# Canleskis/ephemeris-explorer

Measured on AMD Instinct MI355X. Metric: body-steps/s, higher is better.
Workload: dtype f64

## Files before the change

ephemeris_explorer_amd/build.py:

```python
import os
import subprocess
import sys
from pathlib import Path

HERE = Path(__file__).resolve().parent
CSRC = HERE / "csrc"
LIB = HERE / "libephemeris_amd.so"
HOOKS_LIB = HERE / "libephemeris_amd_testhooks.so"
HOOKS_SOURCES = ["debug_api.cpp", "debug_kernels.hip"]
N_PAIR_VARIANTS = 7
PAIR_SOURCES = ["step_wg.hip", "step_wave.hip", "step_small.hip", "step_double_small.hip", "step_srkn_small.hip", "fast.hip", "craft_sweep.hip"]
SOURCES = ["solout.hip", "double_step.hip", "craft.hip", "craft_events.hip", "ephemeris_table.hip", "evaluators.hip", "craft_eval.hip", "craft_restart.hip", "craft_gather.hip", "craft_plot.hip", "craft_markers.hip", "craft_separation.hip", "peer.hip", "dispatch.cpp", "mem.cpp", "coeffs.cpp", "nbody.cpp", "propagator.cpp", "shard.cpp", "api.cpp"]
EXPORTS = CSRC / "exports.map"
HEADERS = sorted(p.name for pat in ("*.h", "*.inc", "exports.map") for p in CSRC.glob(pat)) + ["../../include/ephemeris_amd.h"]
FLAGS = ["--offload-arch=gfx950", "-O3", "-std=c++17", "-fPIC", "-ffp-contract=off", "-fno-fast-math", "-fvisibility=hidden",
         "-Wall", "-Wno-unused-function", "-Wno-unused-result"]
FLAGS += os.environ.get("EPH_EXTRA_FLAGS", "").split()


def hipcc():
    for c in (os.environ.get("HIPCC"), "/opt/rocm/bin/hipcc", "hipcc"):
        if c and (os.path.isabs(c) and os.path.exists(c) or not os.path.isabs(c)):
            return c
    return "hipcc"


def units():
    out = [(src, CSRC / (src.rsplit(".", 1)[0] + ".o"), []) for src in SOURCES + HOOKS_SOURCES]
    for k in range(N_PAIR_VARIANTS):
        out += [(src, CSRC / (src.rsplit(".", 1)[0] + f".pv{k}.o"), [f"-DEPH_PAIR_VARIANT={k}"]) for src in PAIR_SOURCES]
    return out


def needs_build(lib=LIB):
    if not lib.exists():
        return True
    t = lib.stat().st_mtime
    return any((CSRC / f).stat().st_mtime > t for f in SOURCES + HOOKS_SOURCES + PAIR_SOURCES + HEADERS) or Path(__file__).stat().st_mtime > t


def build(force=False, verbose=False, lib=LIB, extra_flags=(), obj_dir=None, jobs=None):
    hooks = lib.with_name(lib.name.replace("libephemeris_amd", "libephemeris_amd_testhooks")) if lib == LIB else None
    if not force and not extra_flags and not needs_build(lib) and (hooks is None or not needs_build(hooks)):
        return lib
    from concurrent.futures import ThreadPoolExecutor
    newest_header = max((CSRC / h).stat().st_mtime for h in HEADERS)
    newest_header = max(newest_header, Path(__file__).stat().st_mtime)
    todo, objs = [], []
    for src, obj, fl in units():
        if obj_dir is not None:
            obj = Path(obj_dir) / obj.name
        objs.append(str(obj))
        if force or extra_flags or not obj.exists() or obj.stat().st_mtime < max((CSRC / src).stat().st_mtime, newest_header):
            todo.append((src, obj, fl))

    def compile_one(job):
        src, obj, fl = job
        cmd = [hipcc(), *FLAGS, *fl, *extra_flags, "-x", "hip", "-c", str(CSRC / src), "-o", str(obj)]
        if verbose:
            print(" ".join(cmd), file=sys.stderr)
        p = subprocess.run(cmd, stdout=subprocess.PIPE, stderr=subprocess.STDOUT)
        if p.returncode:
            raise RuntimeError(f"hipcc failed on {src} {' '.join(fl)}:\n{p.stdout.decode()}")
        if verbose and p.stdout:
            print(p.stdout.decode(), file=sys.stderr)

    todo.sort(key=lambda j: -(CSRC / j[0]).stat().st_size)
    with ThreadPoolExecutor(jobs or max(2, (os.cpu_count() or 4))) as ex:
        list(ex.map(compile_one, todo))
    hook_objs = [o for o in objs if Path(o).name in {h.rsplit(".", 1)[0] + ".o" for h in HOOKS_SOURCES}]
    link = [hipcc(), "--offload-arch=gfx950", "-shared", "-fPIC", f"-Wl,--version-script={EXPORTS}"]
    if hooks is not None:
        subprocess.check_call([*link, "-o", str(lib), *[o for o in objs if o not in hook_objs]])
        subprocess.check_call([*link, "-o", str(hooks), *objs])
    else:
        subprocess.check_call([*link, "-o", str(lib), *objs])
    return lib


def build_all(force=False, verbose=False):
    return [build(force, verbose), HOOKS_LIB]


if __name__ == "__main__":
    if "--exp" in sys.argv:
        i = sys.argv.index("--exp")
        name, flags = sys.argv[i + 1], sys.argv[i + 2:]
        od = Path("/tmp") / f"eph_exp_{name}"
        od.mkdir(parents=True, exist_ok=True)
        print(build(force=True, verbose=False, lib=HERE / f"libephemeris_amd_exp_{name}.so", extra_flags=flags, obj_dir=od))
    else:
        print(build(force="--force" in sys.argv, verbose="--verbose" in sys.argv))
```

ephemeris_explorer_amd/csrc/step_wg.hip:

```cpp
#include <algorithm>
#include <type_traits>
#include <utility>

#include "pair_ns.h"

#ifndef EPH_EXPERIMENTS
#define EPH_EXPERIMENTS 0
#endif
#if !EPH_EXPERIMENTS || !defined(EPH_WG_SIDE)
#undef EPH_WG_SIDE
#define EPH_WG_SIDE 0
#endif
#if !EPH_EXPERIMENTS || !defined(EPH_WG_ABLATE)
#undef EPH_WG_ABLATE
#define EPH_WG_ABLATE 0
#endif
#define WG_LOOP_BARRIER() do { if constexpr (!(EPH_WG_ABLATE & 2)) __syncthreads(); } while (0)


namespace eph {
namespace EPH_PV_NS {

constexpr int kWgBodies = 16;
constexpr int kDuoThreads = 64 * 6;
constexpr int kDuoTailWave = 5;
constexpr int kWgChainWave = 4;
constexpr int kWgTailWave = 8;
constexpr int kWgThreads = 64 * 12;
constexpr int kWgTileBufs = 6;
constexpr int kWgSplitBufs = 3;

template <int NB, int BS = 1, typename PosPtr>
__device__ __forceinline__ void wg_load_own(PosPtr pos, int n, int first, double (&xi)[NB], double (&yi)[NB], double (&zi)[NB]) {
#pragma unroll
    for (int b = 0; b < NB; ++b) {
        const int ii = min(first + BS * b, n - 1);
        xi[b] = pos[ii].x;
        yi[b] = pos[ii].y;
        zi[b] = pos[ii].z;
    }
}
template <typename PosPtr>
__device__ __forceinline__ Body4 load_src(PosPtr pos, int n, int tiles, int lane, int t) {
    const int j = min(t, tiles - 1) * kTile + lane;
    return pos[j < n ? j : n - 1];
}

template <int NB>
__device__ __forceinline__ void wg_pair_tile(const double (&xi)[NB], const double (&yi)[NB], const double (&zi)[NB],
                                             const Body4 &pj, bool ieee, double *tile, int b0, int lane) {
    PairPre pre[NB];
    unsigned worst = ieee ? kRangeSpan : mu_key(pj.mu), low = ~0u;
#pragma unroll
    for (int b = 0; b < NB; ++b) {
        pre[b] = pair_pre(xi[b], yi[b], zi[b], pj);
        worst = max(worst, range_key(pre[b].n2));
        low = min(low, pre[b].lo);
    }
    worst = max(worst, low_key(low));
    double c[3 * NB];
    if (__builtin_amdgcn_ballot_w64(worst >= kRangeSpan) == 0) {
#pragma unroll
        for (int b = 0; b < NB; ++b) pair_finish<true>(pre[b], pj.mu, c[3 * b], c[3 * b + 1], c[3 * b + 2]);
    } else {
#pragma unroll
        for (int b = 0; b < NB; ++b) pair_finish<false>(pre[b], pj.mu, c[3 * b], c[3 * b + 1], c[3 * b + 2]);
    }
#pragma unroll
    for (int q = 0; q < 3 * NB; ++q) {
        if constexpr (EPH_WG_ABLATE & 1) asm volatile("" ::"v"(c[q]));
        else tile[(3 * b0 + q) * kRow + lane] = c[q];
    }
}

template <int NB, typename PosPtr>
__device__ __forceinline__ void wg_pair_wave(PosPtr pos, int n, int i0, int b0, double *C, int lane, int tiles, int tdiag, int wbuf) {
    double xi[NB], yi[NB], zi[NB];
    wg_load_own<NB>(pos, n, i0 + b0, xi, yi, zi);
    Body4 pj = load_src(pos, n, tiles, lane, 0);
    Body4 pjn = load_src(pos, n, tiles, lane, 1);
    wg_pair_tile<NB>(xi, yi, zi, pj, tdiag == 0, C, b0, lane);
    pj = pjn;
    pjn = load_src(pos, n, tiles, lane, 2);
    if (tiles > 1) wg_pair_tile<NB>(xi, yi, zi, pj, tdiag == 1, C + wbuf, b0, lane);
    __syncthreads();
    for (int t = 0; t < tiles; ++t) {
        if (t + 2 < tiles) {
            pj = pjn;
            pjn = load_src(pos, n, tiles, lane, t + 3);
            wg_pair_tile<NB>(xi, yi, zi, pj, tdiag == t + 2, C + ((t + 2) % kWgSplitBufs) * wbuf, b0, lane);
        }
        __syncthreads();
    }
}

template <int NB>
__device__ __forceinline__ void wg_pair_tile2(const double (&xi)[NB], const double (&yi)[NB], const double (&zi)[NB],
                                              const Body4 &pa, const Body4 &pb, bool ieee, double *tile_a, double *tile_b,
                                              int b0, int lane) {
    PairPre pre[2 * NB];
    unsigned worst = ieee ? kRangeSpan : max(mu_key(pa.mu), mu_key(pb.mu)), low = ~0u;
#pragma unroll
    for (int b = 0; b < NB; ++b) {
        pre[b] = pair_pre(xi[b], yi[b], zi[b], pa);
        pre[NB + b] = pair_pre(xi[b], yi[b], zi[b], pb);
        worst = max(worst, max(range_key(pre[b].n2), range_key(pre[NB + b].n2)));
        low = min(low, min(pre[b].lo, pre[NB + b].lo));
    }
    worst = max(worst, low_key(low));
    double c[6 * NB];
    if (__builtin_amdgcn_ballot_w64(worst >= kRangeSpan) == 0) {
        if constexpr (kPairStaged) {
            double mus[2 * NB];
#pragma unroll
            for (int b = 0; b < NB; ++b) { mus[b] = pa.mu; mus[NB + b] = pb.mu; }
            pair_finish_staged<2 * NB>(pre, mus, c);
        } else {
#pragma unroll
            for (int b = 0; b < NB; ++b) {
                pair_finish<true>(pre[b], pa.mu, c[3 * b], c[3 * b + 1], c[3 * b + 2]);
                pair_finish<true>(pre[NB + b], pb.mu, c[3 * (NB + b)], c[3 * (NB + b) + 1], c[3 * (NB + b) + 2]);
            }
        }
    } else {
#pragma unroll
        for (int b = 0; b < NB; ++b) {
            pair_finish<false>(pre[b], pa.mu, c[3 * b], c[3 * b + 1], c[3 * b + 2]);
            pair_finish<false>(pre[NB + b], pb.mu, c[3 * (NB + b)], c[3 * (NB + b) + 1], c[3 * (NB + b) + 2]);
        }
    }
#pragma unroll
    for (int q = 0; q < 3 * NB; ++q) {
        if constexpr (EPH_WG_ABLATE & 1) {
            asm volatile("" ::"v"(c[q]), "v"(c[3 * NB + q]));
        } else {
            tile_a[(3 * b0 + q) * kRow + lane] = c[q];
            tile_b[(3 * b0 + q) * kRow + lane] = c[3 * NB + q];
        }
    }
}

__device__ __forceinline__ int big_start(int K) { return K < 2 ? K : 2 * K - 2; }
__device__ __forceinline__ int big_count(int tiles) { return tiles <= 2 ? tiles : 2 + (tiles - 2 + 1) / 2; }
template <int NB, typename PosPtr>
__device__ __forceinline__ void wg_pair_wave_big(PosPtr pos, int n, int i0, int b0, double *C, int lane, int tiles, int tdiag, int wbuf) {
    double xi[NB], yi[NB], zi[NB];
#pragma unroll
    for (int b = 0; b < NB; ++b) {
        const int ii = min(i0 + b0 + b, n - 1);
        xi[b] = pos[ii].x;
        yi[b] = pos[ii].y;
        zi[b] = pos[ii].z;
    }
    auto produce = [&](int K, const Body4 &pa, const Body4 &pb) {
        const int t = big_start(K);
        if (t >= tiles || EPH_WG_SIDE == 2) return;
        double *ta = C + (t % kWgTileBufs) * wbuf, *tb = C + ((t + 1) % kWgTileBufs) * wbuf;
        if (K >= 2 && t + 1 < tiles) wg_pair_tile2<NB>(xi, yi, zi, pa, pb, tdiag == t || tdiag == t + 1, ta, tb, b0, lane);
        else wg_pair_tile<NB>(xi, yi, zi, pa, tdiag == t, ta, b0, lane);
    };
    const int TB = big_count(tiles);
    Body4 pa = load_src(pos, n, tiles, lane, 0), pb = load_src(pos, n, tiles, lane, 1);
    Body4 na = load_src(pos, n, tiles, lane, 2), nb = load_src(pos, n, tiles, lane, 3);
    produce(0, pa, pa);
    produce(1, pb, pb);
    __syncthreads();
    for (int K = 0; K < TB; ++K) {
        pa = na; pb = nb;
        na = load_src(pos, n, tiles, lane, big_start(K + 3));
        nb = load_src(pos, n, tiles, lane, big_start(K + 3) + 1);
        produce(K + 2, pa, pb);
        WG_LOOP_BARRIER();
    }
}
__device__ __forceinline__ void wg_idle_wave(int tiles) {
    __syncthreads();
    for (int T = 0; T < big_count(tiles); ++T) WG_LOOP_BARRIER();
}

constexpr bool kWgLateThird = kPairVariant == 0 || kPairVariant == 4 || kPairVariant == 5;
static_assert(kWgTileBufs == 6, "the late third tile needs tile t + 6 to be written two intervals after tile t was read");
__device__ __forceinline__ int phase_start(int P) { return P < 2 ? P : 3 * P - 4; }
__device__ __forceinline__ int phase_count(int tiles) { return tiles <= 2 ? tiles : 2 + (tiles - 2 + 2) / 3; }
__device__ __forceinline__ int phase_tiles(int P, int tiles) { return P < 2 ? 1 : min(3, tiles - phase_start(P)); }
__device__ __forceinline__ int interval_count(int tiles) { return phase_count(tiles) + (kWgLateThird && tiles >= 5 && (tiles - 2) % 3 == 0); }
__device__ __forceinline__ int chain_first(int I) { return kWgLateThird ? (I <= 2 ? I : 3 * I - 5) : phase_start(I); }

template <int MA, int MB>
__device__ __forceinline__ void pair_finish_staged_split(const PairPre (&pre)[MA + MB], const double (&mu)[MA + MB], double (&c)[3 * (MA + MB)]) {
    PairPre pa[MA], pb[MB];
    double ma[MA], mb[MB], ca[3 * MA], cb[3 * MB];
#pragma unroll
    for (int k = 0; k < MA; ++k) { pa[k] = pre[k]; ma[k] = mu[k]; }
#pragma unroll
    for (int k = 0; k < MB; ++k) { pb[k] = pre[MA + k]; mb[k] = mu[MA + k]; }
    pair_finish_staged<MA>(pa, ma, ca);
    pair_finish_staged<MB>(pb, mb, cb);
#pragma unroll
    for (int k = 0; k < 3 * MA; ++k) c[k] = ca[k];
#pragma unroll
    for (int k = 0; k < 3 * MB; ++k) c[3 * MA + k] = cb[k];
}

template <int NB, int BS>
__device__ __forceinline__ void wg_store_held(double *tile, int b0, int lane, const double (&held)[3 * NB]) {
#pragma unroll
    for (int q = 0; q < 3 * NB; ++q) {
        if constexpr (EPH_WG_ABLATE & 1) asm volatile("" ::"v"(held[q]));
        else tile[(3 * (b0 + BS * (q / 3)) + q % 3) * kRow + lane] = held[q];
    }
}

template <int NB, int NT, int BS = 1, bool LATE = false>
__device__ __forceinline__ void wg_pair_block(const double (&xi)[NB], const double (&yi)[NB], const double (&zi)[NB],
                                              const Body4 (&pj)[NT], bool ieee, double *const (&tile)[NT], int b0, int lane,
                                              double (&held)[3 * NB], double *held_tile) {
    constexpr int M = NB * NT;
    if constexpr (LATE) wg_store_held<NB, BS>(held_tile, b0, lane, held);
    PairPre pre[M];
    double mus[M];
    unsigned worst = ieee ? kRangeSpan : 0u, low = ~0u;
#pragma unroll
    for (int s = 0; s < NT; ++s) {
        worst = max(worst, mu_key(pj[s].mu));
#pragma unroll
        for (int b = 0; b < NB; ++b) {
            const int k = s * NB + b;
            pre[k] = pair_pre(xi[b], yi[b], zi[b], pj[s]);
            mus[k] = pj[s].mu;
            worst = max(worst, range_key(pre[k].n2));
            low = min(low, pre[k].lo);
        }
    }
    worst = max(worst, low_key(low));
    double c[3 * M];
    if (__builtin_amdgcn_ballot_w64(worst >= kRangeSpan) == 0) {
        if constexpr (kPairStaged && M == 5 && (kPairVariant == 4 || kPairVariant == 6)) {
            pair_finish_staged_split<3, 2>(pre, mus, c);
        } else if constexpr (kPairStaged) {
            pair_finish_staged<M>(pre, mus, c);
        } else {
#pragma unroll
            for (int k = 0; k < M; ++k) pair_finish<true>(pre[k], mus[k], c[3 * k], c[3 * k + 1], c[3 * k + 2]);
        }
    } else {
#pragma unroll
        for (int k = 0; k < M; ++k) pair_finish<false>(pre[k], mus[k], c[3 * k], c[3 * k + 1], c[3 * k + 2]);
    }
#pragma unroll
    for (int s = 0; s < NT - LATE; ++s) {
#pragma unroll
        for (int q = 0; q < 3 * NB; ++q) {
            if constexpr (EPH_WG_ABLATE & 1) asm volatile("" ::"v"(c[3 * NB * s + q]));
            else tile[s][(3 * (b0 + BS * (q / 3)) + q % 3) * kRow + lane] = c[3 * NB * s + q];
        }
    }
    if constexpr (LATE) {
#pragma unroll
        for (int q = 0; q < 3 * NB; ++q) held[q] = c[3 * NB * (NT - 1) + q];
    }
}
template <int NB, int NT, int BS = 1>
__device__ __forceinline__ void wg_pair_block(const double (&xi)[NB], const double (&yi)[NB], const double (&zi)[NB],
                                              const Body4 (&pj)[NT], bool ieee, double *const (&tile)[NT], int b0, int lane) {
    double none[3 * NB];
    wg_pair_block<NB, NT, BS, false>(xi, yi, zi, pj, ieee, tile, b0, lane, none, nullptr);
}

template <int NB, int BS = 1, typename PosPtr>
__device__ __forceinline__ void wg_pair_wave_deal(PosPtr pos, int n, int i0, int b0, int rank, double *C, int lane, int tiles, int tdiag, int wbuf) {
    double xi[NB], yi[NB], zi[NB];
    wg_load_own<NB, BS>(pos, n, i0 + b0, xi, yi, zi);
    auto tile_of = [&](int P) { return P < 2 ? (rank == 0 ? P : tiles) : phase_start(P) + rank; };
    constexpr bool kOff = EPH_WG_SIDE == 2 || (EPH_WG_SIDE == 3 && BS == 1);
    const int NI = interval_count(tiles);
    [[maybe_unused]] const int NP = kWgLateThird ? phase_count(tiles) : NI;
    if constexpr (NB == 5 || !kWgLateThird) {
        auto produce = [&](int t, const Body4 &pj) {
            if (t >= tiles || kOff) return;
            const Body4 src[1] = {pj};
            double *const dst[1] = {C + (t % kWgTileBufs) * wbuf};
            wg_pair_block<NB, 1, BS>(xi, yi, zi, src, t == tdiag, dst, b0, lane);
        };
        Body4 pj = load_src(pos, n, tiles, lane, tile_of(0)), pjn = load_src(pos, n, tiles, lane, tile_of(1));
        produce(tile_of(0), pj);
        __syncthreads();
        for (int P = 1; P < NP; ++P) {
            pj = pjn;
            pjn = load_src(pos, n, tiles, lane, tile_of(P + 1));
            produce(tile_of(P), pj);
            WG_LOOP_BARRIER();
        }
        if (NI > NP) WG_LOOP_BARRIER();
    } else {
        static_assert(NB < 5, "the late loop is the rank-2 waves' (four bodies) and wave 8's (three)");
        double held[3 * NB];
#pragma unroll
        for (int q = 0; q < 3 * NB; ++q) held[q] = 0.0;
        int tprev = tile_of(2);
        Body4 pj, pjn = load_src(pos, n, tiles, lane, tile_of(2));
        __syncthreads();
        for (int I = 1; I < NI; ++I) {
            const int t = I < 2 ? tiles : tile_of(I);
            if (I >= 2) {
                pj = pjn;
                pjn = load_src(pos, n, tiles, lane, tile_of(I + 1));
            }
            double *const late = C + (tprev % kWgTileBufs) * wbuf;
            if (kOff) {
            } else if (t < tiles) {
                const Body4 src[1] = {pj};
                double *const dst[1] = {nullptr};
                wg_pair_block<NB, 1, BS, true>(xi, yi, zi, src, t == tdiag, dst, b0, lane, held, late);
                tprev = t;
            } else if (tprev < tiles && I > 2) {
                wg_store_held<NB, BS>(late, b0, lane, held);
                tprev = tiles;
            }
            WG_LOOP_BARRIER();
        }
    }
}
template <typename PosPtr>
__device__ __forceinline__ void wg_pair_wave_solo(PosPtr pos, int n, int i0, double *C, int lane, int tiles, int tdiag, int wbuf) {
    double xi[1], yi[1], zi[1];
    wg_load_own<1>(pos, n, i0, xi, yi, zi);
    auto load_phase = [&](int P, Body4 (&s)[3]) {
        const int t = phase_start(P);
        s[0] = load_src(pos, n, tiles, lane, t);
        if (P >= 2) { s[1] = load_src(pos, n, tiles, lane, t + 1); s[2] = load_src(pos, n, tiles, lane, t + 2); }
    };
    const int NI = interval_count(tiles), NP = kWgLateThird ? phase_count(tiles) : NI;
    double held[3] = {0.0, 0.0, 0.0};
    int tprev = tiles;
    auto write_held = [&]() {
        if (tprev >= tiles) return;
        double *const late = C + (tprev % kWgTileBufs) * wbuf;
        wg_store_held<1, 1>(late, 0, lane, held);
        tprev = tiles;
    };
    auto produce = [&](int P, const Body4 (&s)[3]) {
        if (EPH_WG_SIDE == 2) return;
        if (P >= NP) { write_held(); return; }
        const int t = phase_start(P), cnt = phase_tiles(P, tiles);
        if (cnt == 3) {
            double *const dst[3] = {C + (t % kWgTileBufs) * wbuf, C + ((t + 1) % kWgTileBufs) * wbuf,
                                    kWgLateThird ? nullptr : C + ((t + 2) % kWgTileBufs) * wbuf};
            const bool below = tdiag < t + 3, own = tdiag >= t && below;
            double *const late = C + ((tprev < tiles ? tprev : t + 2) % kWgTileBufs) * wbuf;
            wg_pair_block<1, 3, 1, kWgLateThird>(xi, yi, zi, s, own, dst, 0, lane, held, late);
            if constexpr (kWgLateThird) tprev = t + 2;
        } else {
            write_held();
            auto one = [&](int k, const Body4 &pj) {
                const Body4 src[1] = {pj};
                double *const dst[1] = {C + ((t + k) % kWgTileBufs) * wbuf};
                wg_pair_block<1, 1>(xi, yi, zi, src, tdiag == t + k, dst, 0, lane);
            };
            one(0, s[0]);
            if (cnt > 1) one(1, s[1]);
        }
    };
    Body4 s[3], sn[3];
    load_phase(0, s);
    load_phase(1, sn);
    produce(0, s);
    __syncthreads();
    for (int P = 1; P < NI; ++P) {
#pragma unroll
        for (int k = 0; k < 3; ++k) s[k] = sn[k];
        load_phase(P + 1, sn);
        produce(P, s);
        WG_LOOP_BARRIER();
    }
}

__device__ __forceinline__ double chain_full_q(const double *row, double2 (&q)[4][8], double acc) {
    load_chunk(row, 2, q[2]);
    acc = add_chunk(q[0], acc);
    load_chunk(row, 3, q[3]);
    acc = add_chunk(q[1], acc);
    acc = add_chunk(q[2], acc);
    return add_chunk(q[3], acc);
}
__device__ __forceinline__ double chain_full_pf(const double *row, const double *row_next, double2 (&q)[4][8],
                                                double acc) {
    load_chunk(row, 2, q[2]);
    acc = add_chunk(q[0], acc);
    load_chunk(row, 3, q[3]);
    acc = add_chunk(q[1], acc);
    load_chunk(row_next, 0, q[0]);
    acc = add_chunk(q[2], acc);
    load_chunk(row_next, 1, q[1]);
    return add_chunk(q[3], acc);
}

constexpr bool wg_tile_split(int wb) { return wb == 4; }
constexpr int wg_split_wave_b(int wb) { return wb == 8 ? 11 : 6; }
template <int WB>
__device__ __forceinline__ int wg_small_body(int wave) {
    if constexpr (WB == 8) {
        switch (wave) { case 1: return 0; case 2: return 1; case 3: return 2; case 5: return 3; case 6: return 4; case 7: return 5;
                        case 9: return 6; case 10: return 7; default: return -1; }
    } else {
        switch (wave) { case 1: return 0; case 2: return 1; case 3: return 2; case 5: return 3; default: return -1; }
    }
}
template <int WB, typename PosPtr>
__device__ __forceinline__ double wg_force_split(PosPtr pos, int n, int i0, double init, double *C, int tid) {
    constexpr int kRows = 3 * WB, kBuf = kRows * kRow;
    const int lane = tid & 63, wave = tid >> 6;
    const int tiles = (n + kTile - 1) / kTile;
    const int tdiag = i0 / kTile;
    double *H = C + kWgSplitBufs * kBuf;
    const int body = wg_small_body<WB>(wave);
    if (body >= 0) { wg_pair_wave<1>(pos, n, i0, body, C, lane, tiles, tdiag, kBuf); return 0.0; }
    const bool isA = wave == kWgChainWave, isB = wave == wg_split_wave_b(WB);
    if (!isA && !isB) { for (int t = 0; t <= tiles; ++t) __syncthreads(); return 0.0; }
    const int ch = lane < kRows ? lane : kRows - 1;
    const double *row = C + ch * kRow;
    const int gself = (i0 % kTile) / WB;
    const int li = (i0 % kTile) + ch / 3;
    double acc = init, accL = 0.0;
    double2 q[4][8];
    auto plain = [&](int t) { return t < tiles && t != tdiag && min(kTile, n - t * kTile) == kTile; };
    auto preload = [&](int t) {
        const double *r = row + (t % kWgSplitBufs) * kBuf;
        load_chunk(r, 0, q[0]); load_chunk(r, 1, q[1]); load_chunk(r, 2, q[2]); load_chunk(r, 3, q[3]);
    };
    __syncthreads();
    if (isA && plain(0)) preload(0);
    for (int t = 0; t < tiles; ++t) {
        const bool mine = ((t & 1) != 0) == isB;
        if (mine) {
            if (t > 0) { acc = H[lane]; accL = H[64 + lane]; }
            if (plain(t)) {
                acc = add_chunk(q[0], acc); acc = add_chunk(q[1], acc); acc = add_chunk(q[2], acc); acc = add_chunk(q[3], acc);
            } else {
                chain_masked<WB>(row + (t % kWgSplitBufs) * kBuf, min(kTile, n - t * kTile), t == tdiag ? gself : -1, li, acc, accL);
            }
            H[lane] = acc;
            H[64 + lane] = accL;
        } else if (plain(t + 1)) {
            preload(t + 1);
        }
        __syncthreads();
    }
    return isA ? H[64 + lane] + H[lane] : 0.0;
}

constexpr int kWgShedFirst = 5, kWgShedStride = 5, kWgShedBodies = 3;
template <typename PosPtr>
__device__ __forceinline__ void wg_tail_wave_phases(PosPtr pos, int n, int i0, double *C, int lane, int tiles, int tdiag, int wbuf) {
    wg_pair_wave_deal<kWgShedBodies, kWgShedStride>(pos, n, i0, kWgShedFirst, 2, C, lane, tiles, tdiag, wbuf);
}


template <int WB = kWgBodies, bool DUO = false, typename PosPtr, std::enable_if_t<WB == kWgBodies && !DUO, int> = 0>
__device__ __forceinline__ double wg_force(PosPtr pos, int n, int i0, double init, double *C, int tid) {
    constexpr int kRows = 3 * WB, kBuf = kRows * kRow;
    const int lane = tid & 63, wave = tid >> 6;
    const int tiles = (n + kTile - 1) / kTile;
    const int tdiag = i0 / kTile;
    const int w = __builtin_amdgcn_readfirstlane(wave);
    if (w == 0) { wg_pair_wave_solo(pos, n, i0, C, lane, tiles, tdiag, kBuf); return 0.0; }
    if ((w & 3) && w < 8) { wg_pair_wave_deal<5>(pos, n, i0, 5 * (w & 3) - 4, w >> 2, C, lane, tiles, tdiag, kBuf); return 0.0; }
    if (w & 3) { wg_pair_wave_deal<4>(pos, n, i0, 5 * (w & 3) - 4, 2, C, lane, tiles, tdiag, kBuf); return 0.0; }
    if (w == kWgTailWave) { wg_tail_wave_phases(pos, n, i0, C, lane, tiles, tdiag, kBuf); return 0.0; }
    const int ch = lane < kRows ? lane : kRows - 1;
    const double *row = C + ch * kRow;
    const int gself = (i0 % kTile) / WB;
    const int li = (i0 % kTile) + ch / 3;
    double acc = init, accL = 0.0;
    double2 q[4][8];
    __builtin_amdgcn_s_setprio(3);
    const int NP = interval_count(tiles);
    __syncthreads();
    for (int P = 0; P < NP; ++P) {
        const int t0 = chain_first(P), nt = min(chain_first(P + 1), tiles) - t0;
        const bool whole = nt == 3 && (tdiag < t0 || tdiag > t0 + 2) && n - (t0 + 2) * kTile >= kTile;
        if constexpr (EPH_WG_SIDE == 1) {
        } else if (whole) {
            const double *r0 = row + (t0 % kWgTileBufs) * kBuf, *r1 = row + ((t0 + 1) % kWgTileBufs) * kBuf;
            const double *r2 = row + ((t0 + 2) % kWgTileBufs) * kBuf;
            load_chunk(r0, 0, q[0]);
            load_chunk(r0, 1, q[1]);
            acc = chain_full_pf(r0, r1, q, acc);
            acc = chain_full_pf(r1, r2, q, acc);
            acc = chain_full_q(r2, q, acc);
        } else {
            for (int t = t0; t < t0 + nt; ++t) {
                const double *r = row + (t % kWgTileBufs) * kBuf;
                const int cnt = min(kTile, n - t * kTile);
                if (t != tdiag && cnt == kTile) { acc = chain_full(r, acc); continue; }
                int lit = li;
                asm volatile("" : "+v"(lit));
                chain_masked<WB>(r, cnt, t == tdiag ? gself : -1, lit, acc, accL);
            }
        }
        if (P + 1 < NP) WG_LOOP_BARRIER();
    }
    return accL + acc;
}

template <int WB, bool DUO = false, typename PosPtr, std::enable_if_t<WB != kWgBodies || DUO, int> = 0>
__device__ __forceinline__ double wg_force(PosPtr pos, int n, int i0, double init, double *C, int tid) {
    constexpr int kRows = 3 * WB, kBuf = kRows * kRow;
    const int lane = tid & 63, wave = tid >> 6;
    const int tiles = (n + kTile - 1) / kTile;
    const int tdiag = i0 / kTile;
    if constexpr (DUO) {
        static_assert(WB == 8, "the duo form is the 8-body workgroup with two bodies per pair wave");
        const int w = __builtin_amdgcn_readfirstlane(wave);
        if (w < 4) { wg_pair_wave_big<2>(pos, n, i0, 2 * w, C, lane, tiles, tdiag, kBuf); return 0.0; }
        if (w == kDuoTailWave) { wg_idle_wave(tiles); return 0.0; }
    } else if constexpr (wg_tile_split(WB)) {
        return wg_force_split<WB>(pos, n, i0, init, C, tid);
    } else {
        const int body = wg_small_body<WB>(wave);
        if (body >= 0) { wg_pair_wave_big<1>(pos, n, i0, body, C, lane, tiles, tdiag, kBuf); return 0.0; }
        if (wave != kWgChainWave) { wg_idle_wave(tiles); return 0.0; }
    }
    const int ch = lane < kRows ? lane : kRows - 1;
    const double *row = C + ch * kRow;
    const int gself = (i0 % kTile) / WB;
    const int li = (i0 % kTile) + ch / 3;
    double acc = init, accL = 0.0;
    double2 q[4][8];
    if constexpr (DUO) __builtin_amdgcn_s_setprio(3);
    const int TB = big_count(tiles);
    __syncthreads();
    load_chunk(row, 0, q[0]);
    load_chunk(row, 1, q[1]);
    for (int T = 0; T < TB; ++T) {
#pragma unroll
        for (int hf = 0; hf < 2; ++hf) {
            const int t = big_start(T) + hf;
            if (t >= tiles || (T < 2 && hf)) break;
            const double *r = row + (t % kWgTileBufs) * kBuf;
            const double *rn = row + ((t + 1) % kWgTileBufs) * kBuf;
            const int cnt = min(kTile, n - t * kTile);
            if constexpr (EPH_WG_SIDE == 1) {
            } else if (t != tdiag && cnt == kTile) {
                acc = chain_full_pf(r, rn, q, acc);
            } else {
                chain_masked<WB>(r, cnt, t == tdiag ? gself : -1, li, acc, accL);
                load_chunk(rn, 0, q[0]);
                load_chunk(rn, 1, q[1]);
            }
        }
        WG_LOOP_BARRIER();
    }
    return accL + acc;
}

constexpr int wg_lds_doubles(int wb, bool duo = false) { return (wg_tile_split(wb) && !duo ? kWgSplitBufs * 3 * wb * kRow + 128 : kWgTileBufs * 3 * wb * kRow); }

template <int WB = kWgBodies>
__global__ void __launch_bounds__(kWgThreads) k_accel_wg(int n, int npad, const Body4 *__restrict__ pos,
                                                         const double *__restrict__ acc_init, double *__restrict__ acc_out,
                                                         int lo, int hi, KickDrift kd) {
    __shared__ __attribute__((aligned(16))) double C[wg_lds_doubles(WB)];
    const int tid = threadIdx.x, lane = tid & 63;
    const int i0 = lo + blockIdx.x * WB;
    const int my_i = i0 + lane / 3, cc = lane % 3;
    const bool owner = (tid >> 6) == kWgChainWave && lane < 3 * WB && my_i < hi;
    const double init = (owner && acc_init) ? acc_init[cc * npad + my_i] : 0.0;
    const double a = wg_force<WB>(pos, n, i0, init, C, tid);
    if (owner) {
        acc_out[cc * npad + my_i] = a;
        if (kd.v) kick_drift_one(kd, (size_t)cc * npad + my_i, my_i, cc, a);
    }
}

template <int L, int WB = kWgBodies, bool DUO = false>
__global__ void __launch_bounds__(DUO ? kDuoThreads : kWgThreads) __attribute__((amdgpu_waves_per_eu(3, 3)))
k_lm_step_wg(const LmArgs a) {
    constexpr int kRows = 3 * WB;
    __shared__ __attribute__((aligned(16))) double C[wg_lds_doubles(WB, DUO)];
    const int tid = threadIdx.x, lane = tid & 63;
    const bool chain_wave = (tid >> 6) == kWgChainWave;
    const bool tail_wave = __builtin_amdgcn_readfirstlane(tid >> 6) == (DUO ? kDuoTailWave : kWgTailWave);
    const int i0 = a.lo + blockIdx.x * WB;
    const int cb = lane / 3, cc = lane % 3;
    const int my_i = i0 + cb;
    const bool owner = tail_wave && lane < kRows && my_i < a.hi;
    const size_t lvl = (size_t)3 * a.npad;
    const size_t off = (size_t)cc * a.npad + (owner ? my_i : 0);
    if (tail_wave) {
        double yv[L], av[L];
#pragma unroll
        for (int j = 0; j < L; ++j) {
            const int slot = (a.cur + j) % L;
            yv[j] = a.Y[slot * lvl + off];
            av[j] = j > 0 ? a.A[slot * lvl + off] : 0.0;
        }
        const int tiles = (a.n + kTile - 1) / kTile;
        if constexpr (wg_tile_split(WB) && !DUO) {
            for (int t = 0; t <= tiles; ++t) __syncthreads();
        } else if constexpr (WB == kWgBodies && !DUO) {
            wg_tail_wave_phases(a.pos_cur, a.n, i0, C, lane, tiles, i0 / kTile, 3 * WB * kRow);
        } else {
            wg_idle_wave(tiles);
        }
        __syncthreads();
        if (owner) {
            const double anew = C[lane];
            a.A[(size_t)a.cur * lvl + off] = anew;
            {
                double prev[L];
#pragma unroll
                for (int j = 0; j < L - 1; ++j) prev[j] = av[j + 1];
                prev[L - 1] = 0.0;
                a.V[off] = lm_cowell<L>(anew, prev, yv[0], yv[1], a.cw, a.h, a.hc);
            }
            maybe_sample(a.samp, my_i, cc, a.step, yv[0]);
            if (a.do_predict) {
                av[0] = anew;
                const double ynext = lm_predict<L>(yv, av, a.wa, a.wb, a.hh);
                const int nslot = (a.cur + L - 1) % L;
                a.Y[(size_t)nslot * lvl + off] = ynext;
                reinterpret_cast<double *>(a.pos_next + my_i)[cc] = ynext;
            }
        }
    } else {
        const double anew = wg_force<WB, DUO>(a.pos_cur, a.n, i0, 0.0, C, tid);
        if (chain_wave && lane < kRows) C[lane] = anew;
        __syncthreads();
    }
}

int accel_wg(hipStream_t s, int wb, int n, int npad, const Body4 *pos, const double *acc_init, double *acc_out, int lo, int hi,
             const KickDrift &kd) {
    const dim3 grid((hi - lo + wb - 1) / wb), block(kWgThreads);
    if (wb == 8) hipLaunchKernelGGL(k_accel_wg<8>, grid, block, 0, s, n, npad, pos, acc_init, acc_out, lo, hi, kd);
    else if (wb == 4) hipLaunchKernelGGL(k_accel_wg<4>, grid, block, 0, s, n, npad, pos, acc_init, acc_out, lo, hi, kd);
    else hipLaunchKernelGGL(k_accel_wg<16>, grid, block, 0, s, n, npad, pos, acc_init, acc_out, lo, hi, kd);
    return launched("k_accel_wg");
}
int lm_step_wg(hipStream_t s, int wb, const LmArgs &a) {
    if (wb == 9) {
        const dim3 grid((a.hi - a.lo + 7) / 8), block(kDuoThreads);
        if (a.L == 12) hipLaunchKernelGGL((k_lm_step_wg<12, 8, true>), grid, block, 0, s, a);
        else if (a.L == 13) hipLaunchKernelGGL((k_lm_step_wg<13, 8, true>), grid, block, 0, s, a);
        else return EPH_ERR_UNSUPPORTED;
        return launched("k_lm_step_wg (six waves)");
    }
    const dim3 grid((a.hi - a.lo + wb - 1) / wb), block(kWgThreads);
    if (a.L == 12 && wb == 8) hipLaunchKernelGGL((k_lm_step_wg<12, 8>), grid, block, 0, s, a);
    else if (a.L == 13 && wb == 8) hipLaunchKernelGGL((k_lm_step_wg<13, 8>), grid, block, 0, s, a);
    else if (a.L == 12 && wb == 4) hipLaunchKernelGGL((k_lm_step_wg<12, 4>), grid, block, 0, s, a);
    else if (a.L == 13 && wb == 4) hipLaunchKernelGGL((k_lm_step_wg<13, 4>), grid, block, 0, s, a);
    else if (a.L == 12) hipLaunchKernelGGL((k_lm_step_wg<12, 16>), grid, block, 0, s, a);
    else if (a.L == 13) hipLaunchKernelGGL((k_lm_step_wg<13, 16>), grid, block, 0, s, a);
    else return EPH_ERR_UNSUPPORTED;
    return launched("k_lm_step_wg");
}

}
}
```

Measured before the change: 134.1 million.

## Preload hot kernel args into SGPRs and defer tail-wave history loads

Passes the frequently used LmArgs fields (pos_cur, n, lo, hi, npad, cur) as separate leading kernel arguments and compiles step_wg.hip with kernarg preloading of six arguments, so the kernel prologue avoids scalar loads from the kernarg segment. The tail wave's Y/A history loads are moved into a hook that runs after the first source tiles are issued, overlapping their latency with the initial pair computation. It also adds a fixed run of s_nop instructions at entry and optional s_memtime stamp instrumentation, which is off by default. The cost is a larger kernarg block with duplicated fields, plus extra live registers in the tail wave while the history is held.

```diff
diff --git a/ephemeris_explorer_amd/build.py b/ephemeris_explorer_amd/build.py
--- a/ephemeris_explorer_amd/build.py
+++ b/ephemeris_explorer_amd/build.py
@@ -16,6 +16,7 @@
 FLAGS = ["--offload-arch=gfx950", "-O3", "-std=c++17", "-fPIC", "-ffp-contract=off", "-fno-fast-math", "-fvisibility=hidden",
          "-Wall", "-Wno-unused-function", "-Wno-unused-result"]
 FLAGS += os.environ.get("EPH_EXTRA_FLAGS", "").split()
+SOURCE_FLAGS = {"step_wg.hip": ["-mllvm", "-amdgpu-kernarg-preload-count=6"]}
 
 
 def hipcc():
@@ -26,9 +27,10 @@
 
 
 def units():
-    out = [(src, CSRC / (src.rsplit(".", 1)[0] + ".o"), []) for src in SOURCES + HOOKS_SOURCES]
+    out = [(src, CSRC / (src.rsplit(".", 1)[0] + ".o"), SOURCE_FLAGS.get(src, [])) for src in SOURCES + HOOKS_SOURCES]
     for k in range(N_PAIR_VARIANTS):
-        out += [(src, CSRC / (src.rsplit(".", 1)[0] + f".pv{k}.o"), [f"-DEPH_PAIR_VARIANT={k}"]) for src in PAIR_SOURCES]
+        out += [(src, CSRC / (src.rsplit(".", 1)[0] + f".pv{k}.o"), [f"-DEPH_PAIR_VARIANT={k}", *SOURCE_FLAGS.get(src, [])])
+                for src in PAIR_SOURCES]
     return out
 
 
diff --git a/ephemeris_explorer_amd/csrc/step_wg.hip b/ephemeris_explorer_amd/csrc/step_wg.hip
--- a/ephemeris_explorer_amd/csrc/step_wg.hip
+++ b/ephemeris_explorer_amd/csrc/step_wg.hip
@@ -15,6 +15,14 @@
 #undef EPH_WG_ABLATE
 #define EPH_WG_ABLATE 0
 #endif
+#if !EPH_EXPERIMENTS || !defined(EPH_WG_ENTRY_ARGS)
+#undef EPH_WG_ENTRY_ARGS
+#define EPH_WG_ENTRY_ARGS 1
+#endif
+#if !EPH_EXPERIMENTS || !defined(EPH_WG_HIST_AT)
+#undef EPH_WG_HIST_AT
+#define EPH_WG_HIST_AT 1
+#endif
 #define WG_LOOP_BARRIER() do { if constexpr (!(EPH_WG_ABLATE & 2)) __syncthreads(); } while (0)
 
 
@@ -22,6 +30,19 @@
 namespace EPH_PV_NS {
 
 constexpr int kWgBodies = 16;
+
+#if !EPH_EXPERIMENTS || !defined(EPH_WG_STAMPS)
+#undef EPH_WG_STAMPS
+#define EPH_WG_STAMPS 0
+#endif
+#if EPH_WG_STAMPS
+__device__ unsigned long long g_wg_stamps[12][8];
+#define WG_STAMP(k) do { if (blockIdx.x == 7 && (threadIdx.x & 63) == 0) g_wg_stamps[threadIdx.x >> 6][k] = __builtin_amdgcn_s_memtime(); } while (0)
+#define WG_STAMP_DATA(k) do { asm volatile("s_waitcnt vmcnt(0)" ::: "memory"); WG_STAMP(k); } while (0)
+#else
+#define WG_STAMP(k) do {} while (0)
+#define WG_STAMP_DATA(k) do {} while (0)
+#endif
 constexpr int kDuoThreads = 64 * 6;
 constexpr int kDuoTailWave = 5;
 constexpr int kWgChainWave = 4;
@@ -267,8 +288,10 @@
     wg_pair_block<NB, NT, BS, false>(xi, yi, zi, pj, ieee, tile, b0, lane, none, nullptr);
 }
 
-template <int NB, int BS = 1, typename PosPtr>
-__device__ __forceinline__ void wg_pair_wave_deal(PosPtr pos, int n, int i0, int b0, int rank, double *C, int lane, int tiles, int tdiag, int wbuf) {
+struct WgNoHook { __device__ __forceinline__ void operator()() const {} };
+template <int NB, int BS = 1, typename PosPtr, typename Hook = WgNoHook>
+__device__ __forceinline__ void wg_pair_wave_deal(PosPtr pos, int n, int i0, int b0, int rank, double *C, int lane, int tiles, int tdiag, int wbuf,
+                                                  Hook &&hook = Hook{}) {
     double xi[NB], yi[NB], zi[NB];
     wg_load_own<NB, BS>(pos, n, i0 + b0, xi, yi, zi);
     auto tile_of = [&](int P) { return P < 2 ? (rank == 0 ? P : tiles) : phase_start(P) + rank; };
@@ -283,8 +306,13 @@
             wg_pair_block<NB, 1, BS>(xi, yi, zi, src, t == tdiag, dst, b0, lane);
         };
         Body4 pj = load_src(pos, n, tiles, lane, tile_of(0)), pjn = load_src(pos, n, tiles, lane, tile_of(1));
+        if constexpr (EPH_WG_HIST_AT == 1) hook();
+        WG_STAMP_DATA(1);
         produce(tile_of(0), pj);
+        WG_STAMP(2);
         __syncthreads();
+        WG_STAMP(3);
+        if constexpr (EPH_WG_HIST_AT == 2) hook();
         for (int P = 1; P < NP; ++P) {
             pj = pjn;
             pjn = load_src(pos, n, tiles, lane, tile_of(P + 1));
@@ -299,7 +327,12 @@
         for (int q = 0; q < 3 * NB; ++q) held[q] = 0.0;
         int tprev = tile_of(2);
         Body4 pj, pjn = load_src(pos, n, tiles, lane, tile_of(2));
+        if constexpr (EPH_WG_HIST_AT == 1) hook();
+        WG_STAMP_DATA(1);
+        WG_STAMP(2);
         __syncthreads();
+        WG_STAMP(3);
+        if constexpr (EPH_WG_HIST_AT == 2) hook();
         for (int I = 1; I < NI; ++I) {
             const int t = I < 2 ? tiles : tile_of(I);
             if (I >= 2) {
@@ -364,8 +397,11 @@
     Body4 s[3], sn[3];
     load_phase(0, s);
     load_phase(1, sn);
+    WG_STAMP_DATA(1);
     produce(0, s);
+    WG_STAMP(2);
     __syncthreads();
+    WG_STAMP(3);
     for (int P = 1; P < NI; ++P) {
 #pragma unroll
         for (int k = 0; k < 3; ++k) s[k] = sn[k];
@@ -450,9 +486,10 @@
 }
 
 constexpr int kWgShedFirst = 5, kWgShedStride = 5, kWgShedBodies = 3;
-template <typename PosPtr>
-__device__ __forceinline__ void wg_tail_wave_phases(PosPtr pos, int n, int i0, double *C, int lane, int tiles, int tdiag, int wbuf) {
-    wg_pair_wave_deal<kWgShedBodies, kWgShedStride>(pos, n, i0, kWgShedFirst, 2, C, lane, tiles, tdiag, wbuf);
+template <typename PosPtr, typename Hook = WgNoHook>
+__device__ __forceinline__ void wg_tail_wave_phases(PosPtr pos, int n, int i0, double *C, int lane, int tiles, int tdiag, int wbuf,
+                                                    Hook &&hook = Hook{}) {
+    wg_pair_wave_deal<kWgShedBodies, kWgShedStride>(pos, n, i0, kWgShedFirst, 2, C, lane, tiles, tdiag, wbuf, hook);
 }
 
 
@@ -475,7 +512,9 @@
     double2 q[4][8];
     __builtin_amdgcn_s_setprio(3);
     const int NP = interval_count(tiles);
+    WG_STAMP(2);
     __syncthreads();
+    WG_STAMP(3);
     for (int P = 0; P < NP; ++P) {
         const int t0 = chain_first(P), nt = min(chain_first(P + 1), tiles) - t0;
         const bool whole = nt == 3 && (tdiag < t0 || tdiag > t0 + 2) && n - (t0 + 2) * kTile >= kTile;
@@ -573,40 +612,56 @@
     }
 }
 
+constexpr int kWgEntryPad = 5;
 template <int L, int WB = kWgBodies, bool DUO = false>
 __global__ void __launch_bounds__(DUO ? kDuoThreads : kWgThreads) __attribute__((amdgpu_waves_per_eu(3, 3)))
-k_lm_step_wg(const LmArgs a) {
+k_lm_step_wg(const Body4 *pos_cur_, int n_, int lo_, int hi_, int npad_, int cur_, const LmArgs a) {
     constexpr int kRows = 3 * WB;
+    if constexpr (WB == kWgBodies && !DUO) WG_STAMP(0);
+    const Body4 *const pos_cur = EPH_WG_ENTRY_ARGS ? pos_cur_ : a.pos_cur;
+    const int n = EPH_WG_ENTRY_ARGS ? n_ : a.n, lo = EPH_WG_ENTRY_ARGS ? lo_ : a.lo, hi = EPH_WG_ENTRY_ARGS ? hi_ : a.hi;
+    const int npad = EPH_WG_ENTRY_ARGS ? npad_ : a.npad, cur = EPH_WG_ENTRY_ARGS ? cur_ : a.cur;
     __shared__ __attribute__((aligned(16))) double C[wg_lds_doubles(WB, DUO)];
     const int tid = threadIdx.x, lane = tid & 63;
     const bool chain_wave = (tid >> 6) == kWgChainWave;
     const bool tail_wave = __builtin_amdgcn_readfirstlane(tid >> 6) == (DUO ? kDuoTailWave : kWgTailWave);
-    const int i0 = a.lo + blockIdx.x * WB;
+    const int i0 = lo + blockIdx.x * WB;
     const int cb = lane / 3, cc = lane % 3;
     const int my_i = i0 + cb;
-    const bool owner = tail_wave && lane < kRows && my_i < a.hi;
-    const size_t lvl = (size_t)3 * a.npad;
-    const size_t off = (size_t)cc * a.npad + (owner ? my_i : 0);
+    const bool owner = tail_wave && lane < kRows && my_i < hi;
+    const size_t lvl = (size_t)3 * npad;
+    const size_t off = (size_t)cc * npad + (owner ? my_i : 0);
+#if EPH_EXPERIMENTS && defined(EPH_WG_PAD)
+    asm volatile(".rept %0\n s_nop 0\n .endr" ::"n"(EPH_WG_PAD));
+#else
+    asm volatile(".rept %0\n s_nop 0\n .endr" ::"n"(kWgEntryPad));
+#endif
     if (tail_wave) {
         double yv[L], av[L];
-#pragma unroll
-        for (int j = 0; j < L; ++j) {
-            const int slot = (a.cur + j) % L;
-            yv[j] = a.Y[slot * lvl + off];
-            av[j] = j > 0 ? a.A[slot * lvl + off] : 0.0;
-        }
-        const int tiles = (a.n + kTile - 1) / kTile;
+        auto load_history = [&]() {
+#pragma unroll
+            for (int j = 0; j < L; ++j) {
+                const int slot = (cur + j) % L;
+                yv[j] = a.Y[slot * lvl + off];
+                av[j] = j > 0 ? a.A[slot * lvl + off] : 0.0;
+            }
+        };
+        constexpr bool kPhaseTail = WB == kWgBodies && !DUO;
+        if constexpr (!kPhaseTail || EPH_WG_HIST_AT == 0) load_history();
+        const int tiles = (n + kTile - 1) / kTile;
         if constexpr (wg_tile_split(WB) && !DUO) {
             for (int t = 0; t <= tiles; ++t) __syncthreads();
         } else if constexpr (WB == kWgBodies && !DUO) {
-            wg_tail_wave_phases(a.pos_cur, a.n, i0, C, lane, tiles, i0 / kTile, 3 * WB * kRow);
+            wg_tail_wave_phases(pos_cur, n, i0, C, lane, tiles, i0 / kTile, 3 * WB * kRow, load_history);
         } else {
             wg_idle_wave(tiles);
         }
+        if constexpr (kPhaseTail) WG_STAMP(4);
         __syncthreads();
+        if constexpr (kPhaseTail) WG_STAMP(5);
         if (owner) {
             const double anew = C[lane];
-            a.A[(size_t)a.cur * lvl + off] = anew;
+            a.A[(size_t)cur * lvl + off] = anew;
             {
                 double prev[L];
 #pragma unroll
@@ -618,15 +673,18 @@
             if (a.do_predict) {
                 av[0] = anew;
                 const double ynext = lm_predict<L>(yv, av, a.wa, a.wb, a.hh);
-                const int nslot = (a.cur + L - 1) % L;
+                const int nslot = (cur + L - 1) % L;
                 a.Y[(size_t)nslot * lvl + off] = ynext;
                 reinterpret_cast<double *>(a.pos_next + my_i)[cc] = ynext;
             }
         }
+        if constexpr (kPhaseTail) WG_STAMP(6);
     } else {
-        const double anew = wg_force<WB, DUO>(a.pos_cur, a.n, i0, 0.0, C, tid);
+        const double anew = wg_force<WB, DUO>(pos_cur, n, i0, 0.0, C, tid);
+        if constexpr (WB == kWgBodies && !DUO) WG_STAMP(4);
         if (chain_wave && lane < kRows) C[lane] = anew;
         __syncthreads();
+        if constexpr (WB == kWgBodies && !DUO) WG_STAMP(5);
     }
 }
 
@@ -641,21 +699,28 @@
 int lm_step_wg(hipStream_t s, int wb, const LmArgs &a) {
     if (wb == 9) {
         const dim3 grid((a.hi - a.lo + 7) / 8), block(kDuoThreads);
-        if (a.L == 12) hipLaunchKernelGGL((k_lm_step_wg<12, 8, true>), grid, block, 0, s, a);
-        else if (a.L == 13) hipLaunchKernelGGL((k_lm_step_wg<13, 8, true>), grid, block, 0, s, a);
+        if (a.L == 12) hipLaunchKernelGGL((k_lm_step_wg<12, 8, true>), grid, block, 0, s, a.pos_cur, a.n, a.lo, a.hi, a.npad, a.cur, a);
+        else if (a.L == 13) hipLaunchKernelGGL((k_lm_step_wg<13, 8, true>), grid, block, 0, s, a.pos_cur, a.n, a.lo, a.hi, a.npad, a.cur, a);
         else return EPH_ERR_UNSUPPORTED;
         return launched("k_lm_step_wg (six waves)");
     }
     const dim3 grid((a.hi - a.lo + wb - 1) / wb), block(kWgThreads);
-    if (a.L == 12 && wb == 8) hipLaunchKernelGGL((k_lm_step_wg<12, 8>), grid, block, 0, s, a);
-    else if (a.L == 13 && wb == 8) hipLaunchKernelGGL((k_lm_step_wg<13, 8>), grid, block, 0, s, a);
-    else if (a.L == 12 && wb == 4) hipLaunchKernelGGL((k_lm_step_wg<12, 4>), grid, block, 0, s, a);
-    else if (a.L == 13 && wb == 4) hipLaunchKernelGGL((k_lm_step_wg<13, 4>), grid, block, 0, s, a);
-    else if (a.L == 12) hipLaunchKernelGGL((k_lm_step_wg<12, 16>), grid, block, 0, s, a);
-    else if (a.L == 13) hipLaunchKernelGGL((k_lm_step_wg<13, 16>), grid, block, 0, s, a);
+    if (a.L == 12 && wb == 8) hipLaunchKernelGGL((k_lm_step_wg<12, 8>), grid, block, 0, s, a.pos_cur, a.n, a.lo, a.hi, a.npad, a.cur, a);
+    else if (a.L == 13 && wb == 8) hipLaunchKernelGGL((k_lm_step_wg<13, 8>), grid, block, 0, s, a.pos_cur, a.n, a.lo, a.hi, a.npad, a.cur, a);
+    else if (a.L == 12 && wb == 4) hipLaunchKernelGGL((k_lm_step_wg<12, 4>), grid, block, 0, s, a.pos_cur, a.n, a.lo, a.hi, a.npad, a.cur, a);
+    else if (a.L == 13 && wb == 4) hipLaunchKernelGGL((k_lm_step_wg<13, 4>), grid, block, 0, s, a.pos_cur, a.n, a.lo, a.hi, a.npad, a.cur, a);
+    else if (a.L == 12) hipLaunchKernelGGL((k_lm_step_wg<12, 16>), grid, block, 0, s, a.pos_cur, a.n, a.lo, a.hi, a.npad, a.cur, a);
+    else if (a.L == 13) hipLaunchKernelGGL((k_lm_step_wg<13, 16>), grid, block, 0, s, a.pos_cur, a.n, a.lo, a.hi, a.npad, a.cur, a);
     else return EPH_ERR_UNSUPPORTED;
     return launched("k_lm_step_wg");
 }
 
 }
 }
+
+#if EPH_WG_STAMPS && EPH_PAIR_VARIANT == 0
+extern "C" __attribute__((visibility("default"))) int eph_wg_stamps(unsigned long long *out) {
+    if (hipDeviceSynchronize() != hipSuccess) return 1;
+    return hipMemcpyFromSymbol(out, HIP_SYMBOL(eph::pv0::g_wg_stamps), sizeof(unsigned long long) * 12 * 8) == hipSuccess ? 0 : 1;
+}
+#endif
```

Result: faster. 137.7 million (median of 6 runs) (+2.6%).
